# mcahny/vps

Measured on AMD Instinct MI355X. Metric: frames/sec FuseTrack 1024x2048, higher is better.
Workload: dtype f32-grade: f16x3 split operands (fp16 pair with scaled residual, 22 significand bits) on MFMA, f32 accumulate

## Files before the change

vps_amd/csrc/corr_mfma.hip:

```cpp
#include "conv_common.h"

namespace {

template <int S2, int R, int NCH>
__global__ __launch_bounds__(256)
void corr_mfma_kernel(const float* __restrict__ in1, int ld1, int coff1, const float* __restrict__ in2, int ld2, int coff2,
                      float* __restrict__ out, int out_ld, int out_coff, int N, int H, int W, int act, float slope,
                      int* __restrict__ status) {
    constexpr int MODE = VPS_PREC_F16X3;
    typedef _Float16 h16;
    typedef vec8<h16> x8;
    typedef vec4<h16> x4;
    constexpr int D = 2 * R + 1;
    constexpr int UW = 64;
    constexpr int BWR = 96;
    constexpr int PD = 8;
    static_assert(R <= 16 && NCH % PD == 0, "band inside the four tiles; static register slots");
    constexpr int OP = D + 1;
    __shared__ __attribute__((aligned(16))) h16 As[NCH * 2 * UW * LDS_LDH];
    __shared__ __attribute__((aligned(16))) h16 Bs[2 * 2 * BWR * LDS_LDH];
    __shared__ float Gs[4 * 32 * 32];
    __shared__ float Os[UW * OP];

    const int t = threadIdx.x, lane = t & 63;
    const int wave = __builtin_amdgcn_readfirstlane(t >> 6);
    const int mi = wave >> 1, ni = mi + (wave & 1);
    const int planeW = W / S2, segs = planeW / UW;
    int bid = blockIdx.x;
    const int useg = bid % segs; bid /= segs;
    const int par = bid % S2; bid /= S2;
    const int y = bid % H, n = bid / H;
    const int u0 = useg * UW;

    const __amdgpu_buffer_rsrc_t r1 = make_rsrc(in1, (unsigned)((size_t)N * H * W * ld1 * 4));
    const __amdgpu_buffer_rsrc_t r2 = make_rsrc(in2, (unsigned)((size_t)N * H * W * ld2 * 4));
    float amax = 0.f;

    {
        const int row0 = t >> 3, k4 = t & 7;
#pragma unroll
        for (int c = 0; c < NCH; ++c) {
            f32x4 v[2];
#pragma unroll
            for (int i = 0; i < 2; ++i) {
                const int row = row0 + 32 * i;
                const int x = S2 * (u0 + row) + par;
                v[i] = buffer_load16<f32x4>(r1, (unsigned)(((size_t)(n * H + y) * W + x) * ld1 + coff1 + 32 * c + 4 * k4) * 4u, 0u);
            }
#pragma unroll
            for (int i = 0; i < 2; ++i) {
                const int row = row0 + 32 * i;
                x4 sp[2];
                split_act<MODE>(v[i], sp, amax);
#pragma unroll
                for (int p = 0; p < 2; ++p)
                    *reinterpret_cast<x4*>(&As[((c * 2 + p) * UW + row) * LDS_LDH + (((k4 >> 1) ^ lds_swz(row)) << 3) + ((k4 & 1) << 2)]) = sp[p];
            }
        }
    }

    unsigned bcol[3];
#pragma unroll
    for (int i = 0; i < 3; ++i) {
        const int e = t + 256 * i, row = e >> 3, k4 = e & 7;
        const int u = u0 - 16 + row;
        bcol[i] = (unsigned)u < (unsigned)planeW ? (unsigned)((size_t)(S2 * u + par) * ld2 + coff2 + 4 * k4) * 4u : 0xFFFFFFF0u;
    }
    f32x4 breg[PD][3];
    auto issue = [&](const int slot, const int tj, const int c) {
        const int y2 = y + (tj - R) * S2;
        const bool rowok = tj < D && (unsigned)y2 < (unsigned)H;
        const unsigned rowoff = rowok ? (unsigned)((size_t)(n * H + y2) * W * ld2) * 4u + (unsigned)c * 128u : 0u;
#pragma unroll
        for (int i = 0; i < 3; ++i)
            breg[slot][i] = buffer_load16<f32x4>(r2, (rowok && bcol[i] != 0xFFFFFFF0u) ? rowoff + bcol[i] : 0xFFFFFFF0u, 0u);
    };
    auto stage = [&](const int slot, const int buf) {
#pragma unroll
        for (int i = 0; i < 3; ++i) {
            const int e = t + 256 * i, row = e >> 3, k4 = e & 7;
            x4 sp[2];
            split_act<MODE>(breg[slot][i], sp, amax);
#pragma unroll
            for (int p = 0; p < 2; ++p)
                *reinterpret_cast<x4*>(&Bs[((buf * 2 + p) * BWR + row) * LDS_LDH + (((k4 >> 1) ^ lds_swz(row)) << 3) + ((k4 & 1) << 2)]) = sp[p];
        }
    };
#pragma unroll
    for (int c = 0; c < PD; ++c) issue(c, 0, c);

    const int arow = (32 * mi + (lane & 31)) * LDS_LDH, asw = lds_swz(lane & 31);
    const int brow = (32 * ni + (lane & 31)) * LDS_LDH;
    const float invC = 1.0f / (float)(32 * NCH);
    float* __restrict__ gs = &Gs[wave * 1024];

    for (int tj = 0; tj < D; ++tj) {
        f32x16 accm, accc;
#pragma unroll
        for (int r = 0; r < 16; ++r) { accm[r] = 0.f; accc[r] = 0.f; }
#pragma unroll
        for (int c = 0; c < NCH; ++c) {
            const int slot = c % PD, buf = c & 1;
            stage(slot, buf);
            if (c + PD < NCH) issue(slot, tj, c + PD); else issue(slot, tj + 1, c + PD - NCH);
            __syncthreads();
#pragma unroll
            for (int m = 0; m < 2; ++m) {
                const int chunk = (((2 * m + (lane >> 5)) ^ asw) << 3);
                const x8 a0 = *reinterpret_cast<const x8*>(&As[((c * 2 + 0) * UW) * LDS_LDH + arow + chunk]);
                const x8 a1 = *reinterpret_cast<const x8*>(&As[((c * 2 + 1) * UW) * LDS_LDH + arow + chunk]);
                const x8 b0 = *reinterpret_cast<const x8*>(&Bs[((buf * 2 + 0) * BWR) * LDS_LDH + brow + chunk]);
                const x8 b1 = *reinterpret_cast<const x8*>(&Bs[((buf * 2 + 1) * BWR) * LDS_LDH + brow + chunk]);
                accc = __builtin_amdgcn_mfma_f32_32x32x16_f16(b1, a0, accc, 0, 0, 0);
                accc = __builtin_amdgcn_mfma_f32_32x32x16_f16(b0, a1, accc, 0, 0, 0);
                accm = __builtin_amdgcn_mfma_f32_32x32x16_f16(b0, a0, accm, 0, 0, 0);
            }
        }
        const int i = lane & 31;
#pragma unroll
        for (int r = 0; r < 16; ++r) {
            const int j = (r & 3) + 8 * (r >> 2) + 4 * (lane >> 5);
            gs[j * 32 + i] = accm[r] + accc[r] * 0.00048828125f;
        }
        __syncthreads();
        const int joff = i + 16 + 32 * (mi - ni) - R;
        for (int ti = lane >> 5; ti < D; ti += 2) {
            const int j = joff + ti;
            if ((unsigned)j < 32u) Os[(32 * mi + i) * OP + ti] = vps_act(gs[j * 32 + i] * invC, act, slope);
        }
        __syncthreads();
        for (int e = t; e < UW * D; e += 256) {
            const int p = e / D, ti = e - p * D;
            const int x = S2 * (u0 + p) + par;
            out[((size_t)(n * H + y) * W + x) * out_ld + out_coff + tj * D + ti] = Os[p * OP + ti];
        }
    }
    if (status && !(amax <= 65504.f)) atomicOr(status, 1);
}

}

__attribute__((visibility("hidden")))
int vpsi_launch_corr_mfma(const float* in1, int ld1, int coff1, const float* in2, int ld2, int coff2, float* out, int out_ld, int out_coff,
                          int N, int H, int W, int C, int max_disp, int stride2, int act, float slope, int32_t* status, hipStream_t s) {
    static const int mode = getenv("VPS_CORR_MFMA") ? atoi(getenv("VPS_CORR_MFMA")) : 1;
    const bool off = !(mode & (stride2 == 2 ? 1 : 2));
    if (off || C != 256 || (ld1 & 3) || (ld2 & 3) || (coff1 & 3) || (coff2 & 3)) return 0;
    if ((size_t)N * H * W * ld1 * 4 >= 0xFFFFFFF0ull || (size_t)N * H * W * ld2 * 4 >= 0xFFFFFFF0ull) return 0;
    const int r = max_disp / stride2;
    if (stride2 == 2 && r == 10 && W % 128 == 0) {
        const long nb = (long)N * H * 2 * (W / 128);
        hipLaunchKernelGGL((corr_mfma_kernel<2, 10, 8>), dim3((unsigned)nb), dim3(256), 0, s, in1, ld1, coff1, in2, ld2, coff2, out, out_ld, out_coff,
                           N, H, W, act, slope, status);
        return 1;
    }
    if (stride2 == 1 && r == 4 && W % 64 == 0) {
        const long nb = (long)N * H * (W / 64);
        hipLaunchKernelGGL((corr_mfma_kernel<1, 4, 8>), dim3((unsigned)nb), dim3(256), 0, s, in1, ld1, coff1, in2, ld2, coff2, out, out_ld, out_coff,
                           N, H, W, act, slope, status);
        return 1;
    }
    return 0;
}
```

Baseline: 55.36.

## Process two output rows per block in correlation kernel to reuse B tiles

Each block now computes two output rows y and y+S2 at once. Each B tile staged from the second image (the shifted rows) is reused across both rows, so D+1 shifted rows are streamed instead of 2*D, roughly halving B loads and splits per output row. The per-wave Gs scratch is dropped: accumulators are written directly into the output staging area, which aliases the B buffer, and the B staging address is precomputed. In exchange the kernel holds twice the accumulator registers, uses a larger A tile in LDS, and has fewer blocks, which may reduce occupancy.

```diff
diff --git a/vps_amd/csrc/corr_mfma.hip b/vps_amd/csrc/corr_mfma.hip
--- a/vps_amd/csrc/corr_mfma.hip
+++ b/vps_amd/csrc/corr_mfma.hip
@@ -2,35 +2,45 @@
 
 namespace {
 
-template <int S2, int R, int NCH>
-__global__ __launch_bounds__(256)
-void corr_mfma_kernel(const float* __restrict__ in1, int ld1, int coff1, const float* __restrict__ in2, int ld2, int coff2,
-                      float* __restrict__ out, int out_ld, int out_coff, int N, int H, int W, int act, float slope,
-                      int* __restrict__ status) {
+template <int S2>
+__host__ __device__ inline int corr_class_units(const int H, const int k) {
+    const int rows = H > k ? (H - k + S2 - 1) / S2 : 0;
+    return (rows + 1) / 2;
+}
+template <int S2>
+__host__ __device__ inline int corr_units(const int H) {
+    int u = 0;
+    for (int k = 0; k < S2; ++k) u += corr_class_units<S2>(H, k);
+    return u;
+}
+
+constexpr int CORR_UW = 64;
+constexpr int CORR_BWR = 96;
+constexpr int CORR_LDS_HALFS(const int NCH) { return 2 * NCH * 2 * CORR_UW * LDS_LDH + 2 * 2 * CORR_BWR * LDS_LDH; }
+
+template <int S2, int R, int NCH, int NR>
+__device__ __forceinline__
+void corr_mfma_rows(_Float16* As, _Float16* Bs, const float* __restrict__ in1, const int ld1, const int coff1,
+                    const float* __restrict__ in2, const int ld2, const int coff2, float* __restrict__ out, const int out_ld,
+                    const int out_coff, const int N, const int H, const int W, const int act, const float slope,
+                    int* __restrict__ status, const int n, const int y, const int par, const int u0) {
     constexpr int MODE = VPS_PREC_F16X3;
     typedef _Float16 h16;
     typedef vec8<h16> x8;
     typedef vec4<h16> x4;
     constexpr int D = 2 * R + 1;
-    constexpr int UW = 64;
-    constexpr int BWR = 96;
-    constexpr int PD = 8;
+    constexpr int NS = D + NR - 1;
+    constexpr int UW = CORR_UW, BWR = CORR_BWR;
+    constexpr int PD = NR == 2 ? 4 : 8;
     static_assert(R <= 16 && NCH % PD == 0, "band inside the four tiles; static register slots");
     constexpr int OP = D + 1;
-    __shared__ __attribute__((aligned(16))) h16 As[NCH * 2 * UW * LDS_LDH];
-    __shared__ __attribute__((aligned(16))) h16 Bs[2 * 2 * BWR * LDS_LDH];
-    __shared__ float Gs[4 * 32 * 32];
-    __shared__ float Os[UW * OP];
+    static_assert(NR * UW * OP * 4 <= 2 * BWR * LDS_LDH * 2, "the output staging rows fit into B buffer 0");
+    float* Os = reinterpret_cast<float*>(Bs);
 
     const int t = threadIdx.x, lane = t & 63;
     const int wave = __builtin_amdgcn_readfirstlane(t >> 6);
     const int mi = wave >> 1, ni = mi + (wave & 1);
-    const int planeW = W / S2, segs = planeW / UW;
-    int bid = blockIdx.x;
-    const int useg = bid % segs; bid /= segs;
-    const int par = bid % S2; bid /= S2;
-    const int y = bid % H, n = bid / H;
-    const int u0 = useg * UW;
+    const int planeW = W / S2;
 
     const __amdgpu_buffer_rsrc_t r1 = make_rsrc(in1, (unsigned)((size_t)N * H * W * ld1 * 4));
     const __amdgpu_buffer_rsrc_t r2 = make_rsrc(in2, (unsigned)((size_t)N * H * W * ld2 * 4));
@@ -38,23 +48,26 @@
 
     {
         const int row0 = t >> 3, k4 = t & 7;
-#pragma unroll
-        for (int c = 0; c < NCH; ++c) {
-            f32x4 v[2];
-#pragma unroll
-            for (int i = 0; i < 2; ++i) {
-                const int row = row0 + 32 * i;
-                const int x = S2 * (u0 + row) + par;
-                v[i] = buffer_load16<f32x4>(r1, (unsigned)(((size_t)(n * H + y) * W + x) * ld1 + coff1 + 32 * c + 4 * k4) * 4u, 0u);
-            }
-#pragma unroll
-            for (int i = 0; i < 2; ++i) {
-                const int row = row0 + 32 * i;
-                x4 sp[2];
-                split_act<MODE>(v[i], sp, amax);
-#pragma unroll
-                for (int p = 0; p < 2; ++p)
-                    *reinterpret_cast<x4*>(&As[((c * 2 + p) * UW + row) * LDS_LDH + (((k4 >> 1) ^ lds_swz(row)) << 3) + ((k4 & 1) << 2)]) = sp[p];
+#pragma unroll 1
+        for (int q = 0; q < NR; ++q) {
+#pragma unroll
+            for (int c = 0; c < NCH; ++c) {
+                f32x4 v[2];
+#pragma unroll
+                for (int i = 0; i < 2; ++i) {
+                    const int row = row0 + 32 * i;
+                    const int x = S2 * (u0 + row) + par;
+                    v[i] = buffer_load16<f32x4>(r1, (unsigned)(((size_t)(n * H + y + q * S2) * W + x) * ld1 + coff1 + 32 * c + 4 * k4) * 4u, 0u);
+                }
+#pragma unroll
+                for (int i = 0; i < 2; ++i) {
+                    const int row = row0 + 32 * i;
+                    x4 sp[2];
+                    split_act<MODE>(v[i], sp, amax);
+#pragma unroll
+                    for (int p = 0; p < 2; ++p)
+                        *reinterpret_cast<x4*>(&As[(((q * NCH + c) * 2 + p) * UW + row) * LDS_LDH + (((k4 >> 1) ^ lds_swz(row)) << 3) + ((k4 & 1) << 2)]) = sp[p];
+                }
             }
         }
     }
@@ -67,23 +80,24 @@
         bcol[i] = (unsigned)u < (unsigned)planeW ? (unsigned)((size_t)(S2 * u + par) * ld2 + coff2 + 4 * k4) * 4u : 0xFFFFFFF0u;
     }
     f32x4 breg[PD][3];
-    auto issue = [&](const int slot, const int tj, const int c) {
-        const int y2 = y + (tj - R) * S2;
-        const bool rowok = tj < D && (unsigned)y2 < (unsigned)H;
+    auto issue = [&](const int slot, const int s, const int c) {
+        const int y2 = y + (s - R) * S2;
+        const bool rowok = s < NS && (unsigned)y2 < (unsigned)H;
         const unsigned rowoff = rowok ? (unsigned)((size_t)(n * H + y2) * W * ld2) * 4u + (unsigned)c * 128u : 0u;
 #pragma unroll
         for (int i = 0; i < 3; ++i)
             breg[slot][i] = buffer_load16<f32x4>(r2, (rowok && bcol[i] != 0xFFFFFFF0u) ? rowoff + bcol[i] : 0xFFFFFFF0u, 0u);
     };
+    int bst = (t >> 3) * LDS_LDH + ((((t & 7) >> 1) ^ lds_swz(t >> 3)) << 3) + ((t & 1) << 2);
+    asm volatile("" : "+v"(bst));
     auto stage = [&](const int slot, const int buf) {
 #pragma unroll
         for (int i = 0; i < 3; ++i) {
-            const int e = t + 256 * i, row = e >> 3, k4 = e & 7;
             x4 sp[2];
             split_act<MODE>(breg[slot][i], sp, amax);
 #pragma unroll
             for (int p = 0; p < 2; ++p)
-                *reinterpret_cast<x4*>(&Bs[((buf * 2 + p) * BWR + row) * LDS_LDH + (((k4 >> 1) ^ lds_swz(row)) << 3) + ((k4 & 1) << 2)]) = sp[p];
+                *reinterpret_cast<x4*>(&Bs[bst + ((buf * 2 + p) * BWR + 32 * i) * LDS_LDH]) = sp[p];
         }
     };
 #pragma unroll
@@ -92,50 +106,96 @@
     const int arow = (32 * mi + (lane & 31)) * LDS_LDH, asw = lds_swz(lane & 31);
     const int brow = (32 * ni + (lane & 31)) * LDS_LDH;
     const float invC = 1.0f / (float)(32 * NCH);
-    float* __restrict__ gs = &Gs[wave * 1024];
-
-    for (int tj = 0; tj < D; ++tj) {
-        f32x16 accm, accc;
-#pragma unroll
-        for (int r = 0; r < 16; ++r) { accm[r] = 0.f; accc[r] = 0.f; }
+    const int pix = lane & 31;
+    const int tbase = 4 * (lane >> 5) - (pix + 16 + 32 * (mi - ni) - R);
+    float* const orow = Os + (32 * mi + pix) * OP + tbase;
+    auto act_sel = [&](const float v) {
+        const float lo = act == VPS_ACT_LEAKY ? v * slope : 0.f;
+        const float a = v > 0.f ? v : lo;
+        return act == VPS_ACT_NONE ? v : a;
+    };
+
+    for (int s = 0; s < NS; ++s) {
+        f32x16 accm[NR], accc[NR];
+#pragma unroll
+        for (int q = 0; q < NR; ++q)
+#pragma unroll
+            for (int r = 0; r < 16; ++r) { accm[q][r] = 0.f; accc[q][r] = 0.f; }
 #pragma unroll
         for (int c = 0; c < NCH; ++c) {
             const int slot = c % PD, buf = c & 1;
             stage(slot, buf);
-            if (c + PD < NCH) issue(slot, tj, c + PD); else issue(slot, tj + 1, c + PD - NCH);
+            if (c + PD < NCH) issue(slot, s, c + PD); else issue(slot, s + 1, c + PD - NCH);
             __syncthreads();
 #pragma unroll
             for (int m = 0; m < 2; ++m) {
                 const int chunk = (((2 * m + (lane >> 5)) ^ asw) << 3);
-                const x8 a0 = *reinterpret_cast<const x8*>(&As[((c * 2 + 0) * UW) * LDS_LDH + arow + chunk]);
-                const x8 a1 = *reinterpret_cast<const x8*>(&As[((c * 2 + 1) * UW) * LDS_LDH + arow + chunk]);
                 const x8 b0 = *reinterpret_cast<const x8*>(&Bs[((buf * 2 + 0) * BWR) * LDS_LDH + brow + chunk]);
                 const x8 b1 = *reinterpret_cast<const x8*>(&Bs[((buf * 2 + 1) * BWR) * LDS_LDH + brow + chunk]);
-                accc = __builtin_amdgcn_mfma_f32_32x32x16_f16(b1, a0, accc, 0, 0, 0);
-                accc = __builtin_amdgcn_mfma_f32_32x32x16_f16(b0, a1, accc, 0, 0, 0);
-                accm = __builtin_amdgcn_mfma_f32_32x32x16_f16(b0, a0, accm, 0, 0, 0);
-            }
-        }
-        const int i = lane & 31;
-#pragma unroll
-        for (int r = 0; r < 16; ++r) {
-            const int j = (r & 3) + 8 * (r >> 2) + 4 * (lane >> 5);
-            gs[j * 32 + i] = accm[r] + accc[r] * 0.00048828125f;
+#pragma unroll
+                for (int q = 0; q < NR; ++q) {
+                    const x8 a0 = *reinterpret_cast<const x8*>(&As[(((q * NCH + c) * 2 + 0) * UW) * LDS_LDH + arow + chunk]);
+                    const x8 a1 = *reinterpret_cast<const x8*>(&As[(((q * NCH + c) * 2 + 1) * UW) * LDS_LDH + arow + chunk]);
+                    accc[q] = __builtin_amdgcn_mfma_f32_32x32x16_f16(b1, a0, accc[q], 0, 0, 0);
+                    accc[q] = __builtin_amdgcn_mfma_f32_32x32x16_f16(b0, a1, accc[q], 0, 0, 0);
+                    accm[q] = __builtin_amdgcn_mfma_f32_32x32x16_f16(b0, a0, accm[q], 0, 0, 0);
+                }
+            }
+        }
+#pragma unroll
+        for (int q = 0; q < NR; ++q) {
+            if ((unsigned)(s - q) < (unsigned)D) {
+                float* op = orow + q * UW * OP;
+#pragma unroll
+                for (int r = 0; r < 16; ++r) {
+                    const int jr = (r & 3) + 8 * (r >> 2);
+                    if ((unsigned)(jr + tbase) < (unsigned)D) op[jr] = act_sel((accm[q][r] + accc[q][r] * 0.00048828125f) * invC);
+                }
+            }
         }
         __syncthreads();
-        const int joff = i + 16 + 32 * (mi - ni) - R;
-        for (int ti = lane >> 5; ti < D; ti += 2) {
-            const int j = joff + ti;
-            if ((unsigned)j < 32u) Os[(32 * mi + i) * OP + ti] = vps_act(gs[j * 32 + i] * invC, act, slope);
+#pragma unroll
+        for (int q = 0; q < NR; ++q) {
+            const int tj = s - q;
+            if ((unsigned)tj < (unsigned)D) {
+                for (int e = t; e < UW * D; e += 256) {
+                    const int p = e / D, ti = e - p * D;
+                    const int x = S2 * (u0 + p) + par;
+                    out[((size_t)(n * H + y + q * S2) * W + x) * out_ld + out_coff + tj * D + ti] = Os[(q * UW + p) * OP + ti];
+                }
+            }
         }
         __syncthreads();
-        for (int e = t; e < UW * D; e += 256) {
-            const int p = e / D, ti = e - p * D;
-            const int x = S2 * (u0 + p) + par;
-            out[((size_t)(n * H + y) * W + x) * out_ld + out_coff + tj * D + ti] = Os[p * OP + ti];
-        }
     }
     if (status && !(amax <= 65504.f)) atomicOr(status, 1);
+}
+
+template <int S2, int R, int NCH>
+__global__ __launch_bounds__(512)
+void corr_mfma_kernel(const float* __restrict__ in1, int ld1, int coff1, const float* __restrict__ in2, int ld2, int coff2,
+                      float* __restrict__ out, int out_ld, int out_coff, int N, int H, int W, int act, float slope,
+                      int* __restrict__ status) {
+    __shared__ __attribute__((aligned(16))) _Float16 smem[CORR_LDS_HALFS(NCH)];
+    _Float16* const As = smem;
+    _Float16* const Bs = smem + 2 * NCH * 2 * CORR_UW * LDS_LDH;
+    const int segs = W / S2 / CORR_UW, units = corr_units<S2>(H);
+    int bid = blockIdx.x;
+    const int useg = bid % segs; bid /= segs;
+    const int par = bid % S2; bid /= S2;
+    int p = bid % units, k = 0;
+    const int n = bid / units;
+#pragma unroll
+    for (int kk = 0; kk < S2 - 1; ++kk) {
+        const int uk = corr_class_units<S2>(H, kk);
+        if (k == kk && p >= uk) { p -= uk; ++k; }
+    }
+    const int y = k + 2 * S2 * p;
+    if (y + S2 < H)
+        corr_mfma_rows<S2, R, NCH, 2>(As, Bs, in1, ld1, coff1, in2, ld2, coff2, out, out_ld, out_coff, N, H, W, act, slope, status, n, y, par,
+                                      useg * CORR_UW);
+    else
+        corr_mfma_rows<S2, R, NCH, 1>(As, Bs, in1, ld1, coff1, in2, ld2, coff2, out, out_ld, out_coff, N, H, W, act, slope, status, n, y, par,
+                                      useg * CORR_UW);
 }
 
 }
@@ -143,19 +203,20 @@
 __attribute__((visibility("hidden")))
 int vpsi_launch_corr_mfma(const float* in1, int ld1, int coff1, const float* in2, int ld2, int coff2, float* out, int out_ld, int out_coff,
                           int N, int H, int W, int C, int max_disp, int stride2, int act, float slope, int32_t* status, hipStream_t s) {
-    static const int mode = getenv("VPS_CORR_MFMA") ? atoi(getenv("VPS_CORR_MFMA")) : 1;
+    const char* const env = getenv("VPS_CORR_MFMA");
+    const int mode = env ? atoi(env) : 1;
     const bool off = !(mode & (stride2 == 2 ? 1 : 2));
     if (off || C != 256 || (ld1 & 3) || (ld2 & 3) || (coff1 & 3) || (coff2 & 3)) return 0;
     if ((size_t)N * H * W * ld1 * 4 >= 0xFFFFFFF0ull || (size_t)N * H * W * ld2 * 4 >= 0xFFFFFFF0ull) return 0;
     const int r = max_disp / stride2;
     if (stride2 == 2 && r == 10 && W % 128 == 0) {
-        const long nb = (long)N * H * 2 * (W / 128);
+        const long nb = (long)N * corr_units<2>(H) * 2 * (W / 128);
         hipLaunchKernelGGL((corr_mfma_kernel<2, 10, 8>), dim3((unsigned)nb), dim3(256), 0, s, in1, ld1, coff1, in2, ld2, coff2, out, out_ld, out_coff,
                            N, H, W, act, slope, status);
         return 1;
     }
     if (stride2 == 1 && r == 4 && W % 64 == 0) {
-        const long nb = (long)N * H * (W / 64);
+        const long nb = (long)N * corr_units<1>(H) * (W / 64);
         hipLaunchKernelGGL((corr_mfma_kernel<1, 4, 8>), dim3((unsigned)nb), dim3(256), 0, s, in1, ld1, coff1, in2, ld2, coff2, out, out_ld, out_coff,
                            N, H, W, act, slope, status);
         return 1;
```

After: 55.51 (median of 6 runs). Within noise of the previous version (+0.3%).
